# Chlumsky/msdfgen

Measured on AMD Instinct MI355X. Metric: MSDF glyphs/sec (64x64, fp32), higher is better.
Workload: dtype f64

## Files before the change

include/msdfgen_hip.h:

```cpp
#ifndef MSDFGEN_HIP_H
#define MSDFGEN_HIP_H

#include <stddef.h>
#include <stdint.h>

#ifdef __cplusplus
extern "C" {
#endif

#define MSDFHIP_ABI_VERSION 5

#define MSDFHIP_MODE_SDF   1
#define MSDFHIP_MODE_PSDF  2
#define MSDFHIP_MODE_MSDF  3
#define MSDFHIP_MODE_MTSDF 4

#define MSDFHIP_EC_DISABLED       0
#define MSDFHIP_EC_INDISCRIMINATE 1
#define MSDFHIP_EC_EDGE_PRIORITY  2
#define MSDFHIP_EC_EDGE_ONLY      3
#define MSDFHIP_DO_NOT_CHECK_DISTANCE  0
#define MSDFHIP_CHECK_DISTANCE_AT_EDGE 1
#define MSDFHIP_ALWAYS_CHECK_DISTANCE  2

// ... 182 lines not shown
int msdfhip_simulate_8bit_host(float *pixels, int width, int height, int row_stride, int channels);

int msdfhip_set_kernel_timing(int enable);
int msdfhip_kernel_timing(double *avg_ms_distance, double *avg_ms_correction, int *launches, int reset);

int msdfhip_trim(void);

int msdfhip_front_door_devices(int *out, int cap);

int msdfhip_reload_tuning(void);
int msdfhip_debug_wait_profile(unsigned long long *out24, int reset);
int msdfhip_debug_bbcount(unsigned *out, int cap, int reset);
int msdfhip_debug_single_call_phases(double *out8, int reset);

int msdfhip_single_call_fallbacks(unsigned long long *barrier_timeouts, unsigned long long *lost_flags, unsigned long long *refused, int reset);

#define MSDFHIP_ROUTE_DIST_SMALL_SIMPLE      0
#define MSDFHIP_ROUTE_DIST_SMALL_OVERLAP     1
#define MSDFHIP_ROUTE_DIST_ONE_QUAD          2
#define MSDFHIP_ROUTE_DIST_ONE_SINGLE        3
#define MSDFHIP_ROUTE_DIST_LDS_QUAD          4
#define MSDFHIP_ROUTE_DIST_LDS_SINGLE        5
#define MSDFHIP_ROUTE_DIST_GLOBAL_DIRECT     6
#define MSDFHIP_ROUTE_DIST_GLOBAL_PERSISTENT 7
#define MSDFHIP_ROUTE_DIST_FULL_SIMPLE       8
#define MSDFHIP_ROUTE_DIST_UNCULLED          9
#define MSDFHIP_ROUTE_EC_QUERY_HEAVIEST     10
#define MSDFHIP_ROUTE_EC_QUERY_BATCH        11
#define MSDFHIP_ROUTE_EC_WIDE_SLOTS         12
#define MSDFHIP_ROUTE_EC_SLOW_ALL           13
#define MSDFHIP_ROUTE_SIGN_WHOLE_ROWS       14
#define MSDFHIP_ROUTE_SIGN_SPLIT            15
#define MSDFHIP_ROUTE_SIGN_CHUNKED          16
#define MSDFHIP_ROUTE_COUNT                 17
int msdfhip_debug_route_counts(unsigned long long *out, int cap, int reset);

#ifdef __cplusplus
}
#endif
#endif
```

msdfgen_amd/csrc/msdf_capi.hip:

```cpp

#include <hip/hip_runtime.h>

#include <algorithm>
#include <atomic>
#include <chrono>
#include <condition_variable>
#include <cmath>
#include <cstdarg>
#include <cstdio>
#include <cstdlib>
#include <cstring>
#include <deque>
#include <functional>
#include <memory>
#include <mutex>
#include <string>
#include <thread>
#include <vector>

#include <sched.h>

#include "msdf_classplan.hpp"
#include "msdf_hostplan.hpp"
#include "msdf_kernels.hpp"
// ... 11 lines not shown
int fail(int code, const char *fmt, ...) {
    char buf[512];
    va_list ap;
    va_start(ap, fmt);
    vsnprintf(buf, sizeof(buf), fmt, ap);
    va_end(ap);
    tlsError = buf;
    return code;
}


static long long nowNsEarly() { return std::chrono::duration_cast<std::chrono::nanoseconds>(std::chrono::steady_clock::now().time_since_epoch()).count(); }

struct Tuning {
    size_t resLdsBudget;
    long persistentRounds;
    bool serialClasses;
    int querySlotCap, queryLpcContours;
    bool hasQueryLds;
    bool hasQueryPolicy;
    int qpEdgeCost, qpMaxEdges, qpMinCount, qpWideMaxEdges;
    float qpWideLoad, qpWideMeanCount;
    size_t signCap;
    bool pipelineTrace;
    int microbatch;
    int queryStatic;
    int queryGridSteps;
    int queryBatch;
    bool noArgPayloadSingle;
    bool noZeroCopySingle;
    bool noFusedSingle;
    double shareGridFactor;
    long persistentGrid;
    long shortRounds;
    long smallLaunchTiles;
    char devices[256];
    int smallMaxEdges;
    int ldsClassTpw;
    int pipelineDepth;
    bool prepLargeTier;
    int hostThreads;
    long singleSpinLimit;
    bool singleVerbose;
};
std::atomic<const Tuning *> gTuning(NULL);
std::mutex gTuningMutex;
std::vector<Tuning *> gTuningTables;

void readTuning() {
    Tuning &t = *new Tuning;
    const char *env;
    t.resLdsBudget = (env = getenv("MSDFHIP_RES_LDS_BUDGET")) ? (size_t) atol(env) : (size_t) 10*1024;
    t.persistentRounds = (env = getenv("MSDFHIP_PERSISTENT_ROUNDS")) ? atol(env) : 8;
    t.serialClasses = getenv("MSDFHIP_SERIAL_CLASSES") != NULL;
    t.querySlotCap = 160, t.queryLpcContours = 24;
    t.hasQueryLds = (env = getenv("MSDFHIP_QUERY_LDS")) != NULL;
    if (env)
        sscanf(env, "%d,%d", &t.querySlotCap, &t.queryLpcContours);
    t.qpEdgeCost = 150, t.qpMaxEdges = 48, t.qpMinCount = 0x7fffffff, t.qpWideMaxEdges = 128, t.qpWideLoad = 4e8f, t.qpWideMeanCount = 24.f;
    t.hasQueryPolicy = (env = getenv("MSDFHIP_QUERY_POLICY")) != NULL;
    if (env)
        sscanf(env, "%d,%d,%d,%d,%f,%f", &t.qpEdgeCost, &t.qpMaxEdges, &t.qpMinCount, &t.qpWideMaxEdges, &t.qpWideLoad, &t.qpWideMeanCount);
    t.signCap = (env = getenv("MSDFHIP_SIGN_CAP")) ? (size_t) atol(env) : (size_t) 192;
    if (t.signCap < 3)
        t.signCap = 3;
    t.pipelineTrace = getenv("MSDFHIP_PIPELINE_TRACE") != NULL;
    t.microbatch = (env = getenv("MSDFHIP_MICROBATCH")) ? atoi(env) : 256;
    if (t.microbatch < 1)
        t.microbatch = 1;
    t.devices[0] = 0;
    t.queryStatic = (env = getenv("MSDFHIP_QUERY_STATIC")) ? atoi(env) : 2;
    t.queryGridSteps = (env = getenv("MSDFHIP_QUERY_GRID")) ? atoi(env) : 16;
    t.queryBatch = (env = getenv("MSDFHIP_QUERY_BATCH")) && atoi(env) > 0 ? atoi(env) : 1;
    t.noFusedSingle = getenv("MSDFHIP_NO_FUSED_SINGLE") != NULL;
    t.noZeroCopySingle = getenv("MSDFHIP_NO_ZERO_COPY_SINGLE") != NULL;
    t.noArgPayloadSingle = getenv("MSDFHIP_NO_ARG_PAYLOAD_SINGLE") != NULL;
    t.shortRounds = (env = getenv("MSDFHIP_SHORT_ROUNDS")) ? atol(env) : 4;
    t.persistentGrid = (env = getenv("MSDFHIP_PERSISTENT_GRID")) ? atol(env) : 0;
    t.shareGridFactor = (env = getenv("MSDFHIP_SHARE_GRID")) ? atof(env) : 1.33;
    t.smallLaunchTiles = (env = getenv("MSDFHIP_SMALL_LAUNCH_TILES")) ? atol(env) : 8192;
    if ((env = getenv("MSDFHIP_DEVICES")))
        snprintf(t.devices, sizeof(t.devices), "%s", env);
    t.smallMaxEdges = (env = getenv("MSDFHIP_SMALL_MAX_EDGES")) && atoi(env) > 0 ? atoi(env) : 128;
    t.ldsClassTpw = (env = getenv("MSDFHIP_LDS_CLASS_TPW")) && atoi(env) == 1 ? 1 : 4;
    t.pipelineDepth = (env = getenv("MSDFHIP_PIPELINE_DEPTH")) && atoi(env) >= 1 && atoi(env) <= 3 ? atoi(env) : 2;
    t.prepLargeTier = getenv("MSDFHIP_PREP_LARGE_TIER") != NULL;
    t.hostThreads = (env = getenv("MSDFHIP_HOST_THREADS")) && atoi(env) > 0 ? atoi(env) : 0;
    t.singleSpinLimit = (env = getenv("MSDFHIP_SINGLE_SPIN_LIMIT")) && atol(env) > 0 ? atol(env) : 0;
    t.singleVerbose = getenv("MSDFHIP_SINGLE_VERBOSE") != NULL;
    gTuningTables.push_back(&t);
    gTuning.store(&t, std::memory_order_release);
}

const Tuning &tuning() {
    const Tuning *t = gTuning.load(std::memory_order_acquire);
    if (!t) {
        std::lock_guard<std::mutex> lock(gTuningMutex);
        if (!gTuning.load(std::memory_order_acquire))
            readTuning();
        t = gTuning.load(std::memory_order_acquire);
    }
    return *t;
}

std::atomic<unsigned long long> gRouteCounts[MSDFHIP_ROUTE_COUNT];

inline void countRoute(int route) { gRouteCounts[route].fetch_add(1, std::memory_order_relaxed); }

#define HIPCHK(expr) do { hipError_t e_ = (expr); if (e_ != hipSuccess) { (void) hipGetLastError(); return fail(MSDFHIP_ERR_HIP, "%s failed: %s (%s:%d)", #expr, hipGetErrorString(e_), __FILE__, __LINE__); } } while (0)

// ... 99 lines not shown
    WorkBuffer() { }
    WorkBuffer(const WorkBuffer &) = delete;
    WorkBuffer &operator=(const WorkBuffer &) = delete;
    ~WorkBuffer() { release(); }
    void release() {
        if (owned && ptr)
            (void) (PINNED ? pinnedFree(ptr) : hipFree(ptr));
        ptr = NULL, cap = 0, owned = false;
    }
    void borrow(T *p, size_t n) { release(); ptr = p, cap = n; }
    hipError_t ensure(size_t n) {
        if (cap >= n)
            return hipSuccess;
        release();
        const hipError_t e = PINNED ? pinnedAlloc((void **) &ptr, n*sizeof(T)) : hipMalloc((void **) &ptr, n*sizeof(T));
        if (e != hipSuccess) {
            ptr = NULL;
            return e;
        }
        cap = n, owned = true;
        return hipSuccess;
    }
};

struct Workspace {
    int device = 0;
    std::mutex mutex;
    WorkBuffer<float> scratch;
    WorkBuffer<EcCandidate> deferred;
    WorkBuffer<EcGlyphParams> ecParams;
    WorkBuffer<double> gres;
    WorkBuffer<unsigned> workQueue;
    unsigned queueParity = 0;
    WorkBuffer<int> bucket;
    WorkBuffer<int, true> hBucket;
    int bucketKey = -1;
    bool bucketUploaded = false;
    WorkBuffer<int> ecOrder;
    WorkBuffer<int, true> hEcOrder;
    hipEvent_t ecOrderReady = NULL;
    bool ecOrderTried = false;
    hipStream_t sideStream[2] = { NULL, NULL };
    hipEvent_t forkEvent = NULL, joinEvent[2] = { NULL, NULL };

    size_t reservedGlyphs = 0;

    void newGlyphRange() { bucketKey = -1, bucketUploaded = false; }
    void reserveGlyphs(size_t n) {
        bucket.release(), hBucket.release(), ecParams.release();
        reservedGlyphs = n;
        newGlyphRange();
    }
    size_t glyphCapacity(int nGlyphs) const { return std::max(std::max((size_t) (nGlyphs > 0 ? nGlyphs : 0), reservedGlyphs), (size_t) 1); }
    ~Workspace() {
        if (!(scratch.owned || deferred.owned || ecParams.owned || gres.owned || workQueue.owned || bucket.owned || hBucket.owned || ecOrder.owned || hEcOrder.owned ||
              ecOrderReady || forkEvent || sideStream[0] || sideStream[1]))
            return;
        (void) hipSetDevice(device);
        for (int k = 0; k < 2; ++k) {
            if (sideStream[k])
                hipStreamDestroy(sideStream[k]);
            if (joinEvent[k])
                hipEventDestroy(joinEvent[k]);
        }
        if (forkEvent)
            hipEventDestroy(forkEvent);
        if (ecOrderReady)
            hipEventDestroy(ecOrderReady);
    }
};

struct ShapeData {
    int nGlyphs = 0, nContours = 0, nEdges = 0, maxContours = 0, maxEdges = 0;
    int32_t *dGlyphContourOffsets = NULL, *dContourOffsets = NULL;
    double *dPoints = NULL;
    uint8_t *dTypes = NULL, *dColors = NULL;
    EdgeRec *dRecs = NULL;
    int8_t *dWindings = NULL;
    mutable std::vector<int> hContours, hEdges;
    void countMaxima() {
        maxContours = maxEdges = 0;
        for (size_t g = 0; g < hContours.size(); ++g)
            maxContours = std::max(maxContours, hContours[g]), maxEdges = std::max(maxEdges, hEdges[g]);
    }
    void setCounts(const int *contours, const int *edges, int n) {
        hContours.assign(contours, contours+n), hEdges.assign(edges, edges+n);
        countMaxima();
    }
// ... 92 lines not shown
    plan.resBytes = resBytes;
    plan.globalRes = overlap && resBytes+idxBytes > plan.ldsBudget;
    plan.idxBytes = idxBytes;
    plan.listStride = maxEdges;
    plan.bytes = plan.globalRes ? tileListBytes(maxEdges, maxContours, true) : resBytes+idxBytes;
    if (plan.bytes > limit)
        return fail(MSDFHIP_ERR_TOO_COMPLEX, "a glyph has %d contours / %d edges: the survivor lists need %zu B of LDS per wavefront, device limit is %zu B",
                    maxContours, maxEdges, plan.bytes, limit);
    return MSDFHIP_OK;
}

template <class K>
int setLds(K kernel, size_t bytes) {
    if (bytes > 64*1024)
        HIPCHK(hipFuncSetAttribute(reinterpret_cast<const void *>(kernel), hipFuncAttributeMaxDynamicSharedMemorySize, (int) bytes));
    return MSDFHIP_OK;
}

int ensureWorkQueue(const MsdfHipBatch *b, unsigned **out, hipStream_t stream) {
    std::lock_guard<std::mutex> lock(b->work.mutex);
    WorkBuffer<unsigned> &q = b->work.workQueue;
    if (!q.ptr) {
        HIPCHK(q.ensure(64));
        const hipError_t e = hipMemsetAsync(q.ptr, 0, 256, stream);
        if (e != hipSuccess) {
            q.release();
            return fail(MSDFHIP_ERR_HIP, "work queue of the persistent launch: %s", hipGetErrorString(e));
        }
    }
    *out = q.ptr;
    return MSDFHIP_OK;
}

int ensureGres(const MsdfHipBatch *b, size_t bytes, double **out) {
    std::lock_guard<std::mutex> lock(b->work.mutex);
    HIPCHK(b->work.gres.ensure((bytes+sizeof(double)-1)/sizeof(double)));
    *out = b->work.gres.ptr;
    return MSDFHIP_OK;
}

template <int SEL, bool OVERLAP, bool GRES, int TPW_>
void launchDistanceKernel(unsigned grid, size_t lds, hipStream_t stream, const DistanceArgs &a) {
    hipLaunchKernelGGL((k_distance<SEL, OVERLAP, GRES, TPW_>), dim3(grid), dim3(WAVE), lds, stream, a.batch.nGlyphs, a.batch.glyphContourOffsets, a.batch.contourOffsets,
                       a.batch.recs, a.batch.windings, a.glyphs, a.width, a.height, a.tilesX, a.tilesPerGlyph, a.maxEdges, a.dst, a.toScratch, a.blockBase, a.gres,
                       a.gresStride, a.glyphMap, a.nMapped, a.workQueue, a.workItems);
}

template <int SEL, bool OVERLAP, bool GRES, int TPW_ = (GRES ? 1 : (int) QUAD)>
int launchDistance(const MsdfHipBatch *b, const MsdfHipGlyph *dGlyphs, int w, int h, float *dst, int toScratch, const LdsPlan &plan, hipStream_t stream,
                   const int *dGlyphMap = NULL, int nMapped = 0, size_t shareGrid = 0, bool *persistent = NULL) {
    const int tilesX = (w+TILE-1)/TILE, tilesY = (h+TILE-1)/TILE, tiles = tilesX*tilesY;
    if (persistent)
        *persistent = false;
    const int nG = dGlyphMap ? nMapped : b->nGlyphs;
    if (nG == 0)
        return MSDFHIP_OK;
    const int tpw = TPW_;
    const size_t blocks = (size_t) nG*(size_t) ((tiles+tpw-1)/tpw);
    if (blocks > 0x7fffffffull)
        return fail(MSDFHIP_ERR_INVALID, "launch of %zu tile quads exceeds the grid limit; split the batch", blocks);
    int rc = setLds(k_distance<SEL, OVERLAP, GRES, TPW_>, plan.bytes);
    if (rc != MSDFHIP_OK)
        return rc;
    double *gres = NULL;
    size_t chunk = blocks, stride = 0;
    unsigned *queue = NULL;
    DistanceArgs args;
    args.batch = viewOf(b), args.glyphs = dGlyphs, args.width = w, args.height = h, args.tilesX = tilesX, args.tilesPerGlyph = tiles, args.maxEdges = plan.listStride;
    args.dst = dst, args.toScratch = toScratch, args.blockBase = 0, args.gres = NULL, args.gresStride = 0, args.glyphMap = dGlyphMap, args.nMapped = nMapped;
    args.workQueue = NULL, args.workItems = 0;
    if (GRES && OVERLAP && plan.resBytes) {
        stride = plan.resBytes/sizeof(double);
        const size_t slots = (size_t) residentSlots(b->device)*4u*MSDF_DISTANCE_WAVES_PER_SIMD;
        const size_t minRounds = (size_t) tuning().persistentRounds;
        const bool byShare = shareGrid > 0 && shareGrid < slots && blocks > shareGrid;
        if (((minRounds && blocks >= minRounds*slots) || byShare) && blocks < 0xffffffffull-8u*slots) {
            chunk = byShare ? shareGrid : slots;
            if (tuning().persistentGrid > 0 && (size_t) tuning().persistentGrid < chunk)
                chunk = (size_t) tuning().persistentGrid;
            rc = ensureGres(b, chunk*plan.resBytes, &gres);
            if (rc == MSDFHIP_OK)
                rc = ensureWorkQueue(b, &queue, stream);
            if (rc != MSDFHIP_OK)
                return rc;
            std::lock_guard<std::mutex> lock(b->work.mutex);
            queue += b->work.queueParity ? 16 : 0;
            args.gres = gres, args.gresStride = stride, args.workQueue = queue, args.workItems = (unsigned) blocks;
            launchDistanceKernel<SEL, OVERLAP, GRES, TPW_>((unsigned) chunk, plan.bytes, stream, args);
            HIPCHK(hipGetLastError());
            b->work.queueParity ^= 1u;
            if (persistent)
                *persistent = true;
            return MSDFHIP_OK;
        }
        chunk = GRES_WORKSPACE_CAP/plan.resBytes;
        if (chunk < 256)
            chunk = 256;
        if (chunk > blocks)
            chunk = blocks;
        rc = ensureGres(b, chunk*plan.resBytes, &gres);
        if (rc != MSDFHIP_OK)
            return rc;
    }
// ... 245 lines not shown
            return rc;
        HIPCHK(hipEventRecord(b->work.forkEvent, stream));
        if (nRest > 0 && b->plan.nSmall > 0) {
            sRest = b->work.sideStream[0];
            HIPCHK(hipStreamWaitEvent(sRest, b->work.forkEvent, 0));
        }
        if (b->plan.nOne > 0 && (b->plan.nSmall > 0 || nRest > 0)) {
            sOne = b->work.sideStream[1];
            HIPCHK(hipStreamWaitEvent(sOne, b->work.forkEvent, 0));
        }
    }
    int aheadRc = MSDFHIP_OK;
    if (ecAhead && sOne != stream) {
        aheadRc = runCorrection(b, SelTraits<SEL>::NCH, w, h, dGlyphs, NULL, NULL, NULL, *ecAhead, sOne, call, true);
    }
    if (nRest > 0) {
        LdsPlan rest = plan;
        rest.globalRes = true;
        rest.bytes = tileListBytes(maxE, maxC, true);
        size_t shareGrid = 0;
        if (tuning().shareGridFactor > 0 && concurrent) {
            const size_t slots = (size_t) residentSlots(b->device)*4u*MSDF_DISTANCE_WAVES_PER_SIMD;
            shareGrid = (size_t) ((double) slots*b->plan.restShare*tuning().shareGridFactor);
            shareGrid = shareGrid < 256 ? 256 : shareGrid;
        }
        rc = launchDistance<SEL, true, true>(b, dGlyphs, w, h, dst, toScratch, rest, sRest, b->work.bucket.ptr+b->plan.nOne+b->plan.nSmall, nRest, shareGrid, &persistent);
        rc = counted(rc, persistent ? MSDFHIP_ROUTE_DIST_GLOBAL_PERSISTENT : MSDFHIP_ROUTE_DIST_GLOBAL_DIRECT);
    }
    if (rc == MSDFHIP_OK && b->plan.nSmall > 0) {
        const size_t slots = (size_t) residentSlots(b->device)*4u*MSDF_DISTANCE_WAVES_PER_SIMD;
        const bool shortLaunch = classTpw == 1 || (size_t) b->plan.nSmall*(size_t) ((tilesAll+QUAD-1)/QUAD) < (size_t) tuning().shortRounds*slots;
        LdsPlan small;
        rc = planLds(b, SelTraits<SEL>::NCH, true, small, b->plan.smallMaxC, b->plan.smallMaxE, shortLaunch ? 1 : (int) QUAD);
        if (rc == MSDFHIP_OK)
            rc = shortLaunch ? counted(launchDistance<SEL, true, false, 1>(b, dGlyphs, w, h, dst, toScratch, small, stream, b->work.bucket.ptr+b->plan.nOne, b->plan.nSmall),
                                       MSDFHIP_ROUTE_DIST_LDS_SINGLE)
                             : counted(launchDistance<SEL, true, false>(b, dGlyphs, w, h, dst, toScratch, small, stream, b->work.bucket.ptr+b->plan.nOne, b->plan.nSmall),
                                       MSDFHIP_ROUTE_DIST_LDS_QUAD);
    }
    if (rc == MSDFHIP_OK && b->plan.nOne > 0) {
        const size_t slots = (size_t) residentSlots(b->device)*4u*MSDF_SIMPLE_WAVES_PER_SIMD;
        const bool shortLaunch = (size_t) b->plan.nOne*(size_t) ((tilesAll+QUAD-1)/QUAD) < (size_t) tuning().shortRounds*slots;
        LdsPlan simple;
        rc = planLds(b, SelTraits<SEL>::NCH, false, simple, 1, b->plan.oneMaxE, shortLaunch ? 1 : (int) QUAD);
        if (rc == MSDFHIP_OK && shortLaunch) {
            simple.bytes = tileListBytes(b->plan.oneMaxE, 1, true);
            rc = counted(launchDistance<SEL, false, true>(b, dGlyphs, w, h, dst, toScratch, simple, sOne, b->work.bucket.ptr, b->plan.nOne), MSDFHIP_ROUTE_DIST_ONE_SINGLE);
        } else if (rc == MSDFHIP_OK)
            rc = counted(launchDistance<SEL, false, false>(b, dGlyphs, w, h, dst, toScratch, simple, sOne, b->work.bucket.ptr, b->plan.nOne), MSDFHIP_ROUTE_DIST_ONE_QUAD);
    }
    hipError_t joinError = hipSuccess;
    if (sRest != stream) {
        hipError_t e = hipEventRecord(b->work.joinEvent[0], sRest);
        if (e == hipSuccess)
            e = hipStreamWaitEvent(stream, b->work.joinEvent[0], 0);
        joinError = e != hipSuccess ? e : joinError;
    }
    if (sOne != stream) {
        hipError_t e = hipEventRecord(b->work.joinEvent[1], sOne);
        if (e == hipSuccess)
            e = hipStreamWaitEvent(stream, b->work.joinEvent[1], 0);
        joinError = e != hipSuccess ? e : joinError;
    }
    rc = aheadRc != MSDFHIP_OK ? aheadRc : rc;
    if (joinError != hipSuccess) {
        (void) hipGetLastError();
        if (sRest != stream)
            (void) hipStreamSynchronize(sRest);
        if (sOne != stream)
            (void) hipStreamSynchronize(sOne);
        if (rc == MSDFHIP_OK)
// ... 3165 lines not shown
```

msdfgen_amd/csrc/msdf_classplan.hpp:

```cpp

#pragma once

#include <algorithm>
#include <cstddef>

namespace msdfhip {

inline size_t tileListBytes(int maxEdges, int maxContours, bool withBounds) { return ((size_t) maxEdges+(withBounds ? 4 : 1)*(size_t) maxContours+2)*sizeof(int); }

const int SMALL_MAX_EDGES = 128;
const int COST_LDS_MAX_CONTOURS = 5;

inline double glyphCost(int contours, int edges) {
    static const double kOne[4] = { 0.25625, 0.01190, 0.00000, 0.00000 }, kLds[4] = { 0.38398, 0.00846, -0.02755, 0.003446 }, kGlobal[4] = { 1.11611, 0.015776, -0.05039, 0.000681 };
    const double *k = contours <= 1 ? kOne : (contours <= COST_LDS_MAX_CONTOURS && edges <= SMALL_MAX_EDGES) ? kLds : kGlobal;
    const double c = k[0]+k[1]*edges+k[2]*contours+k[3]*(double) edges*contours;
    return c > k[0] ? c : k[0];
}

struct ClassPlan {
    int nOne = 0, nSmall = 0, nHuge = 0;
    int oneMaxE = 0, smallMaxC = 0, smallMaxE = 0, restMaxC = 0, restMaxE = 0;
    float restShare = 1.f;
};

inline ClassPlan planClasses(const int *contours, const int *edges, int n, int limit, int smallMaxEdges, size_t ldsLimit, int *order) {
    auto classOf = [=](int g) {
        if (tileListBytes(edges[g], contours[g], true) > ldsLimit)
            return 3;
        return contours[g] <= 1 ? 0 : contours[g] <= limit && edges[g] <= smallMaxEdges ? 1 : 2;
    };
    int end[4], maxC[4] = { 0, 0, 0, 0 }, maxE[4] = { 0, 0, 0, 0 }, at = 0;
    for (int k = 0; k < 4; ++k) {
        for (int g = 0; g < n; ++g)
            if (classOf(g) == k) {
                order[at++] = g;
                maxC[k] = std::max(maxC[k], contours[g]), maxE[k] = std::max(maxE[k], edges[g]);
            }
        end[k] = at;
    }
    auto heavier = [=](int x, int y) { return (long long) edges[x]*std::max(contours[x], 1) > (long long) edges[y]*std::max(contours[y], 1); };
    for (int k = 0; k < 3; ++k)
        std::stable_sort(order+(k ? end[k-1] : 0), order+end[k], heavier);
    double all = 0, rest = 0;
    for (int g = 0; g < n; ++g)
        all += glyphCost(contours[g], edges[g]);
    for (int k = end[1]; k < end[2]; ++k)
        rest += glyphCost(contours[order[k]], edges[order[k]]);
    ClassPlan p;
    p.nOne = end[0], p.nSmall = end[1]-end[0], p.nHuge = end[3]-end[2];
    p.oneMaxE = maxE[0], p.smallMaxC = maxC[1], p.smallMaxE = maxE[1], p.restMaxC = maxC[2], p.restMaxE = maxE[2];
    p.restShare = all > 0 ? (float) (rest/all) : 1.f;
    return p;
}

}
```

msdfgen_amd/csrc/msdf_kernels.hpp:

```cpp
#pragma once

#include <hip/hip_runtime.h>
#include "msdf_device.hpp"
#include "msdf_prep.hpp"
#include "msdf_ec.hpp"
#include "msdf_ec_fast.hpp"
#include "msdf_cull.hpp"
#include "msdf_scanline.hpp"
#include "msdf_shapeprep.hpp"
#include "msdf_frame.hpp"
#include "../../include/msdfgen_hip.h"

namespace msdfhip {

#ifndef MSDF_DISTANCE_WAVES_PER_SIMD
#define MSDF_DISTANCE_WAVES_PER_SIMD 4
#endif
constexpr int TILE = 8;
constexpr int WAVE = 64;
constexpr int REC_DOUBLES = sizeof(EdgeRec)/sizeof(double);

struct BatchView {
    int nGlyphs;
    const int32_t *glyphContourOffsets;
// ... 112 lines not shown
__device__ inline GlyphWork decodeItem(unsigned b, int nGlyphs, int tilesPerGlyph) {
    GlyphWork w;
    const unsigned fullBlocks = ((unsigned) nGlyphs&~7u)*(unsigned) tilesPerGlyph;
    if (b >= fullBlocks) {
        const unsigned j = b-fullBlocks;
        w.g = (int) (((unsigned) nGlyphs&~7u)+j/(unsigned) tilesPerGlyph);
        w.tile = (int) (j%(unsigned) tilesPerGlyph);
    } else {
        const unsigned xcd = b&7u, slot = b>>3;
        w.g = (int) ((slot/(unsigned) tilesPerGlyph)*8u+xcd);
        w.tile = (int) (slot%(unsigned) tilesPerGlyph);
    }
    w.valid = w.g < nGlyphs;
    return w;
}
__device__ inline GlyphWork decodeBlock(int nGlyphs, int tilesPerGlyph, unsigned blockBase = 0) {
    return decodeItem(blockIdx.x+blockBase, nGlyphs, tilesPerGlyph);
}

__device__ inline unsigned nextItem(unsigned *counters, unsigned total, int &steal) {
    const unsigned x = blockIdx.x&7u;
    while (steal < 8) {
        const unsigned xx = (x+(unsigned) steal)&7u;
        unsigned k = 0;
        if (threadIdx.x == 0)
            k = atomicAdd(&counters[xx], 1u);
        k = (unsigned) __builtin_amdgcn_readfirstlane((int) k);
        const unsigned b = k*8u+xx;
        if (b < total)
            return b;
        ++steal;
    }
    return ~0u;
}

__device__ inline Xform loadXform(const MsdfHipGlyph &gd) {
    Xform t;
    t.sx = gd.xf[0], t.sy = gd.xf[1], t.tx = gd.xf[2], t.ty = gd.xf[3];
    t.mapScale = gd.xf[4], t.mapTranslate = gd.xf[5];
    return t;
}

__device__ inline void stageRecords(double *dst, const EdgeRec *src, int n) {
    const double *s = reinterpret_cast<const double *>(src);
    const int total = n*REC_DOUBLES;
    for (int i = threadIdx.x; i < total; i += blockDim.x)
        dst[i] = s[i];
}


__device__ inline void waveSync() {
    __builtin_amdgcn_fence(__ATOMIC_RELEASE, "wavefront");
    __builtin_amdgcn_wave_barrier();
    __builtin_amdgcn_fence(__ATOMIC_ACQUIRE, "wavefront");
}

__device__ inline float waveMinNonNegative(float v) {
    int x = __float_as_int(v);
    const int inf = 0x7f800000;
#define MSDF_DPP_MIN(ctrl, rowmask) { const int y = __builtin_amdgcn_update_dpp(inf, x, ctrl, rowmask, 0xf, false); x = y < x ? y : x; }
    MSDF_DPP_MIN(0x111, 0xf)
    MSDF_DPP_MIN(0x112, 0xf)
    MSDF_DPP_MIN(0x114, 0xf)
    MSDF_DPP_MIN(0x118, 0xf)
    MSDF_DPP_MIN(0x142, 0xa)
    MSDF_DPP_MIN(0x143, 0xc)
// ... 273 lines not shown
        __syncthreads();
        if (rank == 0)
            for (int r = 1; r < TEAM; ++r) {
                Selector<SEL> other;
                teamGet(other, x+(size_t) (r-1)*TEAM_XCHG_DOUBLES*WAVE, lane);
                selMergePartial(s, other);
            }
        __syncthreads();
        return rank == 0;
    }
    __device__ bool isHelper() const { return rank != 0; }
};

enum { QUAD = 4 };

#ifndef MSDF_SIMPLE_WAVES_PER_SIMD
#define MSDF_SIMPLE_WAVES_PER_SIMD 5
#endif
struct DistanceArgs {
    BatchView batch;
    const MsdfHipGlyph *glyphs;
    int width, height, tilesX, tilesPerGlyph, maxEdges;
    float *dst;
    int toScratch;
    unsigned blockBase;
    double *gres;
    size_t gresStride;
    const int *glyphMap;
    int nMapped;
    unsigned *workQueue;
    unsigned workItems;
};

template <int SEL, bool OVERLAP, bool GRES, int TPW_ = (GRES ? 1 : (int) QUAD), int TEAM = 1>
__device__ __forceinline__ void distanceBody(int nGlyphs, const int32_t *__restrict__ glyphContourOffsets, const int32_t *__restrict__ contourOffsets, const EdgeRec *__restrict__ recs,
           const int8_t *__restrict__ windings, const MsdfHipGlyph *__restrict__ glyphs, int width, int height, int tilesX, int tilesPerGlyph, int maxEdges,
           float *__restrict__ dst, int toScratch, unsigned blockBase, double *__restrict__ gres, size_t gresStride, const int *__restrict__ glyphMap, int nMapped,
           unsigned *__restrict__ workQueue, unsigned workItems, const unsigned blockId, double *smem, const int knownContours = -1, const int knownEdges = -1,
           double *teamXchg = NULL) {
    static_assert(TEAM == 1 || (TPW_ == 1 && !GRES), "teams take one tile, combiner scratch in LDS");
    const int teamRank = TEAM > 1 ? MSDF_UNIFORM((int) (threadIdx.x>>6)) : 0;
    enum { NCH = SelTraits<SEL>::NCH, TPW = TPW_, ROW = WAVE/TPW };
    BatchView batch;
    batch.nGlyphs = nGlyphs, batch.glyphContourOffsets = glyphContourOffsets, batch.contourOffsets = contourOffsets, batch.recs = recs, batch.windings = windings;
    unsigned item = blockId+blockBase;
    int steal = 0;
    const bool persistent = GRES && workQueue != NULL;
    for (;;) {
    if (persistent) {
        item = nextItem(workQueue, workItems, steal);
        if (item == ~0u) {
            if (blockId == 0 && threadIdx.x < 8)
                reinterpret_cast<unsigned *>(reinterpret_cast<size_t>(workQueue)^64u)[threadIdx.x] = 0u;
            return;
        }
    }
    const int quadsPerGlyph = (tilesPerGlyph+TPW-1)/TPW;
    GlyphWork wk = decodeItem(item, glyphMap ? nMapped : batch.nGlyphs, quadsPerGlyph);
    if (!wk.valid)
        return;
    if (glyphMap)
        wk.g = MSDF_UNIFORM(glyphMap[wk.g]);
    const int c0 = knownContours >= 0 ? 0 : MSDF_UNIFORM(batch.glyphContourOffsets[wk.g]), C = knownContours >= 0 ? knownContours : MSDF_UNIFORM(batch.glyphContourOffsets[wk.g+1])-c0;
    const int32_t *coff = batch.contourOffsets+c0;
    const int e0 = knownContours >= 0 ? 0 : MSDF_UNIFORM(coff[0]);
    const int lane = TEAM > 1 ? (int) (threadIdx.x&(WAVE-1)) : (int) threadIdx.x;
    const EdgeRec *rec = batch.recs+e0;

    double *res = GRES ? gres+(size_t) blockId*gresStride : smem;
    int *lists = reinterpret_cast<int *>(smem+(OVERLAP && !GRES ? (size_t) C*NCH*WAVE : 0));
    int *cstarts = lists+(size_t) TPW*maxEdges;

    const MsdfHipGlyph gd = glyphs[wk.g];
    const Xform t = loadXform(gd);
    WindingMasks wind;
    wind.mem = batch.windings+c0;
    if (OVERLAP) {
        const int w = lane < C ? (int) wind.mem[lane] : 0;
        wind.pos = __ballot(w > 0), wind.neg = __ballot(w < 0);
    }
#if defined(MSDF_PROFILE_WAITS)
    MSDF_STAMP(pStart);
    unsigned long long pAcc[16] = { 0, 0, 0, 0, 0, 0, 0, 0, 0, 0, 0, 0, 0, 0, 0, 0 };
#endif

    const double rsx = 1/t.sx, rsy = 1/t.sy;
    const bool fastXf = divSafe(t.sx) && divSafe(t.sy);
    const double hx = (.5*TILE-.5)*fabs(rsx), hy = (.5*TILE-.5)*fabs(rsy);
    const double tr = sqrt(hx*hx+hy*hy);
    if (TEAM == 1 || teamRank == 0) {
        const int q = lane/ROW, col = lane%ROW;
// ... 161 lines not shown
#if defined(__HIP_DEVICE_COMPILE__)
        asm volatile("" : "+v"(laneAfter));
#endif
        const int xo = tx*TILE+(laneAfter&(TILE-1)), yo = ty*TILE+(laneAfter>>3);
        const int yn = gd.flip ? height-1-yo : yo;
        float *px = toScratch ? dst+(((size_t) wk.g*height+yn)*width+xo)*NCH
                              : dst+gd.out_offset+(ptrdiff_t) gd.row_stride*yn+(ptrdiff_t) NCH*xo;
        for (int ch = 0; ch < NCH; ++ch) {
            __builtin_nontemporal_store(mapDistance(t, d[ch]), &px[ch]);
        }
#if defined(MSDF_PROFILE_WAITS)
        {
            MSDF_STAMP(tTile1);
            edges.prof[13] += tTile1-tTile0;
        }
        for (int i = 0; i < 16; ++i)
            pAcc[i] += edges.prof[i];
#endif
    }
#if defined(MSDF_PROFILE_WAITS)
    {
        MSDF_STAMP(pEnd);
        if (lane == 0) {
            atomicAdd(&gWaitProfile[0], 1ull), atomicAdd(&gWaitProfile[1], pEnd-pStart), atomicAdd(&gWaitProfile[2], pPhase2-pStart);
            atomicAdd(&gWaitProfile[3], pAcc[0]), atomicAdd(&gWaitProfile[4], pAcc[1]), atomicAdd(&gWaitProfile[5], pAcc[2]), atomicAdd(&gWaitProfile[6], pAcc[3]);
            atomicAdd(&gWaitProfile[7], pAcc[4]), atomicAdd(&gWaitProfile[8], pAcc[5]), atomicAdd(&gWaitProfile[9], pAcc[6]), atomicAdd(&gWaitProfile[10], pEnd-pPhase2);
            atomicAdd(&gWaitProfile[11], pAcc[7]&0xffffffffull), atomicAdd(&gWaitProfile[12], pAcc[7]>>32);
            atomicAdd(&gWaitProfile[13], pAcc[8]), atomicAdd(&gWaitProfile[14], pAcc[9]), atomicAdd(&gWaitProfile[15], pAcc[10]);
            atomicAdd(&gWaitProfile[16], pAcc[11]), atomicAdd(&gWaitProfile[17], pAcc[13]);
            atomicAdd(&gWaitProfile[18], pAcc[14]), atomicAdd(&gWaitProfile[19], pAcc[15]);
        }
    }
#endif
    if (!persistent)
        return;
    waveSync();
    }
}

template <int SEL, bool OVERLAP, bool GRES = false, int TPW_ = (GRES ? 1 : (int) QUAD)>
__global__ void __launch_bounds__(WAVE, OVERLAP ? MSDF_DISTANCE_WAVES_PER_SIMD : GRES ? MSDF_SIMPLE_WAVES_PER_SIMD-1 : MSDF_SIMPLE_WAVES_PER_SIMD)
k_distance(int nGlyphs, const int32_t *__restrict__ glyphContourOffsets, const int32_t *__restrict__ contourOffsets, const EdgeRec *__restrict__ recs,
           const int8_t *__restrict__ windings, const MsdfHipGlyph *__restrict__ glyphs, int width, int height, int tilesX, int tilesPerGlyph, int maxEdges,
           float *__restrict__ dst, int toScratch, unsigned blockBase, double *__restrict__ gres, size_t gresStride, const int *__restrict__ glyphMap, int nMapped,
           unsigned *__restrict__ workQueue, unsigned workItems) {
    extern __shared__ __attribute__((aligned(16))) double smem[];
    distanceBody<SEL, OVERLAP, GRES, TPW_>(nGlyphs, glyphContourOffsets, contourOffsets, recs, windings, glyphs, width, height, tilesX, tilesPerGlyph, maxEdges, dst, toScratch, blockBase,
                                     gres, gresStride, glyphMap, nMapped, workQueue, workItems, blockIdx.x, smem);
}


template <bool OVERLAP, class Wind = const int8_t *, class Edges = EdgesAll>
struct PsdfQuery {
    const EdgeRec *rec;
    const int32_t *coff;
    Wind windings;
    int C;
    double *res;
    __device__ double operator()(V2 q) const {
        double out[1];
        Edges edges;
        edges.coff = coff;
        if (OVERLAP)
            shapeDistanceOverlap<2>(rec, edges, windings, C, q, res, WAVE, out);
        else
            shapeDistanceSimple<2>(rec, edges, C, q, out);
        return out[0];
    }
};

typedef PB PBSlot;

struct EdgesCooperative {
    const int32_t *coff;
    int lane;
    PBSlot *slots;
    PBSlot *merged;
    int nE, C;
    mutable unsigned long long cached;
    int cacheCap;
// ... 1271 lines not shown
```

msdfgen_amd/lib.py:

```python
import ctypes as C
import os
import threading

import numpy as np

from . import build as _build

MODE_SDF, MODE_PSDF, MODE_MSDF, MODE_MTSDF = 1, 2, 3, 4
CHANNELS = {1: 1, 2: 1, 3: 3, 4: 4}
EC_DISABLED, EC_INDISCRIMINATE, EC_EDGE_PRIORITY, EC_EDGE_ONLY = 0, 1, 2, 3
DO_NOT_CHECK_DISTANCE, CHECK_DISTANCE_AT_EDGE, ALWAYS_CHECK_DISTANCE = 0, 1, 2
FILL_NONZERO, FILL_ODD, FILL_POSITIVE, FILL_NEGATIVE = 0, 1, 2, 3
ERR_NO_DEVICE, ERR_INVALID, ERR_HIP, ERR_TOO_COMPLEX, ERR_NOMEM = -1, -2, -3, -4, -5

_dp = C.POINTER(C.c_double)
_ip = C.POINTER(C.c_int32)
_fp = C.POINTER(C.c_float)
_bp = C.POINTER(C.c_uint8)
_vp = C.c_void_p


class MsdfHipError(RuntimeError):
    def __init__(self, code, message):
        super().__init__("msdfgen_hip error %d: %s" % (code, message))
# ... 84 lines not shown
    "msdfhip_front_door_devices": (C.c_int, [C.POINTER(C.c_int), C.c_int]),
    "msdfhip_debug_wait_profile": (C.c_int, [C.POINTER(C.c_ulonglong), C.c_int]),
    "msdfhip_debug_single_call_phases": (C.c_int, [C.POINTER(C.c_double), C.c_int]),
    "msdfhip_debug_bbcount": (C.c_int, [C.POINTER(C.c_uint32), C.c_int, C.c_int]),
    "msdfhip_generate_stream": (C.c_int, [C.c_int, C.c_int, C.c_int, C.c_int, C.c_int, _vp, _vp, _vp, C.c_size_t, _vp, C.c_size_t, _vp, C.POINTER(Config)]),
    "msdfhip_generate_stream_csr": (C.c_int, [C.c_int, C.c_int, C.c_int, C.c_int, C.c_int, _ip, _ip, _dp, _bp, _bp, _vp, _vp, C.c_size_t, _vp, C.c_size_t, _vp,
                                              C.POINTER(Config)]),
    "msdfhip_generate_stream_prepared": (C.c_int, [C.c_int, C.c_int, C.c_int, C.c_int, C.c_int, _vp, _vp, _vp, C.c_size_t, _vp, C.c_size_t, _vp, C.POINTER(Config),
                                                   C.POINTER(PrepConfig), C.POINTER(C.c_uint64)]),
    "msdfhip_generate_stream_csr_prepared": (C.c_int, [C.c_int, C.c_int, C.c_int, C.c_int, C.c_int, _ip, _ip, _dp, _bp, _bp, _vp, _vp, C.c_size_t, _vp, C.c_size_t,
                                                       _vp, C.POINTER(Config), C.POINTER(PrepConfig), C.POINTER(C.c_uint64)]),
    "msdfhip_generate_stream_prepared_oriented": (C.c_int, [C.c_int, C.c_int, C.c_int, C.c_int, C.c_int, _vp, _vp, _vp, C.c_size_t, _vp, C.c_size_t, _vp,
                                                            C.POINTER(Config), C.POINTER(PrepConfig), C.POINTER(C.c_uint64), C.POINTER(OrientConfig)]),
    "msdfhip_generate_stream_csr_prepared_oriented": (C.c_int, [C.c_int, C.c_int, C.c_int, C.c_int, C.c_int, _ip, _ip, _dp, _bp, _bp, _vp, _vp, C.c_size_t, _vp,
                                                                C.c_size_t, _vp, C.POINTER(Config), C.POINTER(PrepConfig), C.POINTER(C.c_uint64),
                                                                C.POINTER(OrientConfig)]),
    "msdfhip_batch_bounds": (C.c_int, [_vp, _dp]),
    "msdfhip_batch_frame": (C.c_int, [_vp, C.POINTER(FrameConfig), C.c_int, C.c_int, _vp, _vp]),
    "msdfhip_generate_stream_prepared_oriented_framed": (C.c_int, [C.c_int, C.c_int, C.c_int, C.c_int, C.c_int, _vp, _vp, _vp, C.c_size_t, _vp, C.c_size_t, _vp,
                                                                   C.POINTER(Config), C.POINTER(PrepConfig), C.POINTER(C.c_uint64), C.POINTER(OrientConfig),
                                                                   C.POINTER(FrameConfig)]),
    "msdfhip_generate_stream_csr_prepared_oriented_framed": (C.c_int, [C.c_int, C.c_int, C.c_int, C.c_int, C.c_int, _ip, _ip, _dp, _bp, _bp, _vp, _vp, C.c_size_t,
                                                                       _vp, C.c_size_t, _vp, C.POINTER(Config), C.POINTER(PrepConfig), C.POINTER(C.c_uint64),
                                                                       C.POINTER(OrientConfig), C.POINTER(FrameConfig)]),
    "msdfhip_set_host_threads": (C.c_int, [C.c_int]),
    "msdfhip_single_call_fallbacks": (C.c_int, [C.POINTER(C.c_ulonglong), C.POINTER(C.c_ulonglong), C.POINTER(C.c_ulonglong), C.c_int]),
    "msdfhip_debug_route_counts": (C.c_int, [C.POINTER(C.c_ulonglong), C.c_int, C.c_int]),
}

EXPORTED_SYMBOLS = tuple(sorted(_PROTOS))

ROUTE_NAMES = ("dist_small_simple", "dist_small_overlap", "dist_one_quad", "dist_one_single", "dist_lds_quad", "dist_lds_single", "dist_global_direct",
               "dist_global_persistent", "dist_full_simple", "dist_unculled", "ec_query_heaviest", "ec_query_batch", "ec_wide_slots", "ec_slow_all",
               "sign_whole_rows", "sign_split", "sign_chunked")

_lib = None
_lock = threading.Lock()


def library_path():
    return _build.LIB


def load(build_if_missing=True):
    global _lib
    with _lock:
        if _lib is not None:
            return _lib
        try:
            import torch
        except ImportError:
            pass
        path = os.environ.get("MSDFGEN_HIP_LIB") or _build.LIB
        if path == _build.LIB and not os.path.exists(path):
            if not build_if_missing:
                raise MsdfHipError(ERR_NO_DEVICE, "libmsdfgen_hip.so is not built (python -m msdfgen_amd.build)")
            _build.build_lib()
        lib = C.CDLL(path)
        for name, (restype, argtypes) in _PROTOS.items():
            fn = getattr(lib, name)
            fn.restype = restype
            fn.argtypes = argtypes
        if lib.msdfhip_abi_version() != 5:
            raise MsdfHipError(ERR_INVALID, "ABI version mismatch")
        _lib = lib
        return lib

# ... 50 lines not shown
```

Measured before the change: 1.732 million.

## Add glyph-affine persistent scheduling for the LDS quad distance kernel

Adds a persistent launch mode for the LDS-class quad distance kernel. Each wave reads its XCC and CU hardware ids and pulls tiles from per-XCC, per-home-CU atomic counters, so tiles of the same glyph land on the same CU or XCC and reuse its cached edge data. A one-time probe kernel maps the live CU slots to homes, and waves that run out of local work steal from other XCCs using a ballot over counters. In exchange it adds atomic contention, a probe launch on first use, and reliance on hardware register layouts; small launches keep the old path through a round-count threshold.

```diff
diff --git a/include/msdfgen_hip.h b/include/msdfgen_hip.h
--- a/include/msdfgen_hip.h
+++ b/include/msdfgen_hip.h
@@ -238,7 +238,8 @@
 #define MSDFHIP_ROUTE_SIGN_WHOLE_ROWS       14
 #define MSDFHIP_ROUTE_SIGN_SPLIT            15
 #define MSDFHIP_ROUTE_SIGN_CHUNKED          16
-#define MSDFHIP_ROUTE_COUNT                 17
+#define MSDFHIP_ROUTE_DIST_LDS_AFFINE        17
+#define MSDFHIP_ROUTE_COUNT                 18
 int msdfhip_debug_route_counts(unsigned long long *out, int cap, int reset);
 
 #ifdef __cplusplus
diff --git a/msdfgen_amd/csrc/msdf_capi.hip b/msdfgen_amd/csrc/msdf_capi.hip
--- a/msdfgen_amd/csrc/msdf_capi.hip
+++ b/msdfgen_amd/csrc/msdf_capi.hip
@@ -67,6 +67,10 @@
     bool noFusedSingle;
     double shareGridFactor;
     long persistentGrid;
+    int affineMode;
+    long affineRounds;
+    double affineGridFactor;
+    int affineHomeCus;
     long shortRounds;
     long smallLaunchTiles;
     char devices[256];
@@ -111,6 +115,10 @@
     t.noZeroCopySingle = getenv("MSDFHIP_NO_ZERO_COPY_SINGLE") != NULL;
     t.noArgPayloadSingle = getenv("MSDFHIP_NO_ARG_PAYLOAD_SINGLE") != NULL;
     t.shortRounds = (env = getenv("MSDFHIP_SHORT_ROUNDS")) ? atol(env) : 4;
+    t.affineMode = (env = getenv("MSDFHIP_AFFINE")) ? (atoi(env) != 0 ? 1 : 0) : -1;
+    t.affineRounds = (env = getenv("MSDFHIP_AFFINE_ROUNDS")) && atol(env) >= 0 ? atol(env) : 8;
+    t.affineGridFactor = (env = getenv("MSDFHIP_AFFINE_GRID")) && atof(env) > 0 ? atof(env) : 1.0;
+    t.affineHomeCus = (env = getenv("MSDFHIP_AFFINE_HOME")) && !strcmp(env, "pair") ? 2 : 1;
     t.persistentGrid = (env = getenv("MSDFHIP_PERSISTENT_GRID")) ? atol(env) : 0;
     t.shareGridFactor = (env = getenv("MSDFHIP_SHARE_GRID")) ? atof(env) : 1.33;
     t.smallLaunchTiles = (env = getenv("MSDFHIP_SMALL_LAUNCH_TILES")) ? atol(env) : 8192;
@@ -276,6 +284,9 @@
     WorkBuffer<double> gres;
     WorkBuffer<unsigned> workQueue;
     unsigned queueParity = 0;
+    WorkBuffer<unsigned> affineQueue;
+    unsigned affineParity = 0;
+    int affineHomeCus = 0;
     WorkBuffer<int> bucket;
     WorkBuffer<int, true> hBucket;
     int bucketKey = -1;
@@ -297,7 +308,7 @@
     }
     size_t glyphCapacity(int nGlyphs) const { return std::max(std::max((size_t) (nGlyphs > 0 ? nGlyphs : 0), reservedGlyphs), (size_t) 1); }
     ~Workspace() {
-        if (!(scratch.owned || deferred.owned || ecParams.owned || gres.owned || workQueue.owned || bucket.owned || hBucket.owned || ecOrder.owned || hEcOrder.owned ||
+        if (!(scratch.owned || deferred.owned || ecParams.owned || gres.owned || workQueue.owned || affineQueue.owned || bucket.owned || hBucket.owned || ecOrder.owned || hEcOrder.owned ||
               ecOrderReady || forkEvent || sideStream[0] || sideStream[1]))
             return;
         (void) hipSetDevice(device);
@@ -456,6 +467,82 @@
     return MSDFHIP_OK;
 }
 
+struct Placement {
+    int homes[2] = { 0, 0 };
+    uint8_t table[2][AFFINE_PLACEMENT_SLOTS];
+};
+const Placement *placementOf(int device) {
+    static std::mutex mutex;
+    static Placement *known[64];
+    if (device < 0 || device >= 64)
+        return NULL;
+    std::lock_guard<std::mutex> lock(mutex);
+    if (known[device])
+        return known[device];
+    Placement *p = new Placement;
+    known[device] = p;
+    memset(p->table, 0, sizeof(p->table));
+    uint8_t *dSeen = NULL;
+    hipStream_t s = NULL;
+    std::vector<uint8_t> seen((size_t) AFFINE_PLACEMENT_SLOTS, 0);
+    bool ok = hipMalloc((void **) &dSeen, AFFINE_PLACEMENT_SLOTS) == hipSuccess && hipStreamCreateWithFlags(&s, hipStreamNonBlocking) == hipSuccess &&
+              hipMemsetAsync(dSeen, 0, AFFINE_PLACEMENT_SLOTS, s) == hipSuccess;
+    if (ok) {
+        hipLaunchKernelGGL(k_probe_placement, dim3((unsigned) residentSlots(device)*64u), dim3(WAVE), 0, s, dSeen);
+        ok = hipGetLastError() == hipSuccess && hipMemcpyAsync(seen.data(), dSeen, AFFINE_PLACEMENT_SLOTS, hipMemcpyDeviceToHost, s) == hipSuccess &&
+             hipStreamSynchronize(s) == hipSuccess;
+    }
+    if (s)
+        (void) hipStreamDestroy(s);
+    if (dSeen)
+        (void) hipFree(dSeen);
+    if (!ok) {
+        (void) hipGetLastError();
+        return p;
+    }
+    int fewest = AFFINE_MAX_HOMES;
+    for (int x = 0; x < 8; ++x) {
+        int n = 0;
+        for (int k = 0; k < 256; ++k)
+            n += seen[(size_t) x*256+k] != 0;
+        fewest = std::min(fewest, n);
+    }
+    if (fewest < 1)
+        return p;
+    for (int pair = 0; pair < 2; ++pair) {
+        const int H = pair ? (fewest+1)/2 : fewest;
+        for (int x = 0; x < 8; ++x)
+            for (int k = 0, rank = 0; k < 256; ++k) {
+                const bool live = seen[(size_t) x*256+k] != 0;
+                p->table[pair][(size_t) x*256+k] = (uint8_t) ((live ? (pair ? rank/2 : rank) : k)%H);
+                rank += live;
+            }
+        p->homes[pair] = H;
+    }
+    return p;
+}
+
+int ensureAffineQueue(const MsdfHipBatch *b, const Placement *p, int homeCus, unsigned **out, hipStream_t stream) {
+    std::lock_guard<std::mutex> lock(b->work.mutex);
+    WorkBuffer<unsigned> &q = b->work.affineQueue;
+    if (!q.ptr) {
+        HIPCHK(q.ensure(AFFINE_QUEUE_WORDS));
+        b->work.affineHomeCus = 0, b->work.affineParity = 0;
+        const hipError_t e = hipMemsetAsync(q.ptr, 0, sizeof(unsigned)*2*AFFINE_SET_WORDS, stream);
+        if (e != hipSuccess) {
+            q.release();
+            return fail(MSDFHIP_ERR_HIP, "work queues of the glyph-affine launch: %s", hipGetErrorString(e));
+        }
+    }
+    if (b->work.affineHomeCus != homeCus) {
+        HIPCHK(hipMemcpyAsync(q.ptr+2*AFFINE_SET_WORDS, p->table[homeCus == 2], AFFINE_PLACEMENT_SLOTS, hipMemcpyHostToDevice, stream));
+        HIPCHK(hipMemsetAsync(q.ptr, 0, sizeof(unsigned)*2*AFFINE_SET_WORDS, stream));
+        b->work.affineHomeCus = homeCus;
+    }
+    *out = q.ptr;
+    return MSDFHIP_OK;
+}
+
 int ensureGres(const MsdfHipBatch *b, size_t bytes, double **out) {
     std::lock_guard<std::mutex> lock(b->work.mutex);
     HIPCHK(b->work.gres.ensure((bytes+sizeof(double)-1)/sizeof(double)));
@@ -463,9 +550,9 @@
     return MSDFHIP_OK;
 }
 
-template <int SEL, bool OVERLAP, bool GRES, int TPW_>
+template <int SEL, bool OVERLAP, bool GRES, int TPW_, bool AFFINE = false>
 void launchDistanceKernel(unsigned grid, size_t lds, hipStream_t stream, const DistanceArgs &a) {
-    hipLaunchKernelGGL((k_distance<SEL, OVERLAP, GRES, TPW_>), dim3(grid), dim3(WAVE), lds, stream, a.batch.nGlyphs, a.batch.glyphContourOffsets, a.batch.contourOffsets,
+    hipLaunchKernelGGL((k_distance<SEL, OVERLAP, GRES, TPW_, AFFINE>), dim3(grid), dim3(WAVE), lds, stream, a.batch.nGlyphs, a.batch.glyphContourOffsets, a.batch.contourOffsets,
                        a.batch.recs, a.batch.windings, a.glyphs, a.width, a.height, a.tilesX, a.tilesPerGlyph, a.maxEdges, a.dst, a.toScratch, a.blockBase, a.gres,
                        a.gresStride, a.glyphMap, a.nMapped, a.workQueue, a.workItems);
 }
@@ -493,6 +580,26 @@
     args.batch = viewOf(b), args.glyphs = dGlyphs, args.width = w, args.height = h, args.tilesX = tilesX, args.tilesPerGlyph = tiles, args.maxEdges = plan.listStride;
     args.dst = dst, args.toScratch = toScratch, args.blockBase = 0, args.gres = NULL, args.gresStride = 0, args.glyphMap = dGlyphMap, args.nMapped = nMapped;
     args.workQueue = NULL, args.workItems = 0;
+    if (!GRES && OVERLAP && TPW_ == (int) QUAD && shareGrid > 0) {
+        const int homeCus = tuning().affineHomeCus;
+        const Placement *p = placementOf(b->device);
+        const int H = p ? p->homes[homeCus == 2] : 0;
+        if (H > 0 && H <= (int) AFFINE_MAX_HOMES) {
+            rc = ensureAffineQueue(b, p, homeCus, &queue, stream);
+            if (rc == MSDFHIP_OK)
+                rc = setLds(k_distance<SEL, OVERLAP, GRES, TPW_, (!GRES && OVERLAP && TPW_ == (int) QUAD)>, plan.bytes);
+            if (rc != MSDFHIP_OK)
+                return rc;
+            std::lock_guard<std::mutex> lock(b->work.mutex);
+            args.workQueue = queue, args.workItems = (unsigned) H|(b->work.affineParity<<8);
+            launchDistanceKernel<SEL, OVERLAP, GRES, TPW_, (!GRES && OVERLAP && TPW_ == (int) QUAD)>((unsigned) std::min(shareGrid, blocks), plan.bytes, stream, args);
+            HIPCHK(hipGetLastError());
+            b->work.affineParity ^= 1u;
+            if (persistent)
+                *persistent = true;
+            return MSDFHIP_OK;
+        }
+    }
     if (GRES && OVERLAP && plan.resBytes) {
         stride = plan.resBytes/sizeof(double);
         const size_t slots = (size_t) residentSlots(b->device)*4u*MSDF_DISTANCE_WAVES_PER_SIMD;
@@ -804,11 +911,23 @@
         const bool shortLaunch = classTpw == 1 || (size_t) b->plan.nSmall*(size_t) ((tilesAll+QUAD-1)/QUAD) < (size_t) tuning().shortRounds*slots;
         LdsPlan small;
         rc = planLds(b, SelTraits<SEL>::NCH, true, small, b->plan.smallMaxC, b->plan.smallMaxE, shortLaunch ? 1 : (int) QUAD);
-        if (rc == MSDFHIP_OK)
-            rc = shortLaunch ? counted(launchDistance<SEL, true, false, 1>(b, dGlyphs, w, h, dst, toScratch, small, stream, b->work.bucket.ptr+b->plan.nOne, b->plan.nSmall),
-                                       MSDFHIP_ROUTE_DIST_LDS_SINGLE)
-                             : counted(launchDistance<SEL, true, false>(b, dGlyphs, w, h, dst, toScratch, small, stream, b->work.bucket.ptr+b->plan.nOne, b->plan.nSmall),
-                                       MSDFHIP_ROUTE_DIST_LDS_QUAD);
+        if (rc == MSDFHIP_OK && shortLaunch)
+            rc = counted(launchDistance<SEL, true, false, 1>(b, dGlyphs, w, h, dst, toScratch, small, stream, b->work.bucket.ptr+b->plan.nOne, b->plan.nSmall),
+                         MSDFHIP_ROUTE_DIST_LDS_SINGLE);
+        else if (rc == MSDFHIP_OK) {
+            size_t affineGrid = 0;
+            if (tuning().affineMode != 0) {
+                affineGrid = (size_t) ((double) slots*(concurrent ? b->plan.smallShare : 1.f)*tuning().affineGridFactor);
+                affineGrid = std::min(std::max(affineGrid, (size_t) 256), slots);
+                if (tuning().affineMode < 0 && (size_t) b->plan.nSmall*(size_t) ((tilesAll+QUAD-1)/QUAD) < (size_t) tuning().affineRounds*affineGrid)
+                    affineGrid = 0;
+            }
+            bool affine = false;
+            rc = launchDistance<SEL, true, false>(b, dGlyphs, w, h, dst, toScratch, small, stream, b->work.bucket.ptr+b->plan.nOne, b->plan.nSmall, affineGrid, &affine);
+            rc = counted(rc, MSDFHIP_ROUTE_DIST_LDS_QUAD);
+            if (affine)
+                rc = counted(rc, MSDFHIP_ROUTE_DIST_LDS_AFFINE);
+        }
     }
     if (rc == MSDFHIP_OK && b->plan.nOne > 0) {
         const size_t slots = (size_t) residentSlots(b->device)*4u*MSDF_SIMPLE_WAVES_PER_SIMD;
diff --git a/msdfgen_amd/csrc/msdf_classplan.hpp b/msdfgen_amd/csrc/msdf_classplan.hpp
--- a/msdfgen_amd/csrc/msdf_classplan.hpp
+++ b/msdfgen_amd/csrc/msdf_classplan.hpp
@@ -22,6 +22,7 @@
     int nOne = 0, nSmall = 0, nHuge = 0;
     int oneMaxE = 0, smallMaxC = 0, smallMaxE = 0, restMaxC = 0, restMaxE = 0;
     float restShare = 1.f;
+    float smallShare = 1.f;
 };
 
 inline ClassPlan planClasses(const int *contours, const int *edges, int n, int limit, int smallMaxEdges, size_t ldsLimit, int *order) {
@@ -42,15 +43,18 @@
     auto heavier = [=](int x, int y) { return (long long) edges[x]*std::max(contours[x], 1) > (long long) edges[y]*std::max(contours[y], 1); };
     for (int k = 0; k < 3; ++k)
         std::stable_sort(order+(k ? end[k-1] : 0), order+end[k], heavier);
-    double all = 0, rest = 0;
+    double all = 0, rest = 0, small = 0;
     for (int g = 0; g < n; ++g)
         all += glyphCost(contours[g], edges[g]);
     for (int k = end[1]; k < end[2]; ++k)
         rest += glyphCost(contours[order[k]], edges[order[k]]);
+    for (int k = end[0]; k < end[1]; ++k)
+        small += glyphCost(contours[order[k]], edges[order[k]]);
     ClassPlan p;
     p.nOne = end[0], p.nSmall = end[1]-end[0], p.nHuge = end[3]-end[2];
     p.oneMaxE = maxE[0], p.smallMaxC = maxC[1], p.smallMaxE = maxE[1], p.restMaxC = maxC[2], p.restMaxE = maxE[2];
     p.restShare = all > 0 ? (float) (rest/all) : 1.f;
+    p.smallShare = all > 0 ? (float) (small/all) : 1.f;
     return p;
 }
 
diff --git a/msdfgen_amd/csrc/msdf_kernels.hpp b/msdfgen_amd/csrc/msdf_kernels.hpp
--- a/msdfgen_amd/csrc/msdf_kernels.hpp
+++ b/msdfgen_amd/csrc/msdf_kernels.hpp
@@ -168,6 +168,60 @@
         ++steal;
     }
     return ~0u;
+}
+
+enum { AFFINE_MAX_HOMES = 64, AFFINE_COUNTER_WORDS = 16, AFFINE_SET_WORDS = 8*AFFINE_MAX_HOMES*AFFINE_COUNTER_WORDS, AFFINE_PLACEMENT_SLOTS = 8*256,
+       AFFINE_QUEUE_WORDS = 2*AFFINE_SET_WORDS+AFFINE_PLACEMENT_SLOTS/4 };
+
+__device__ inline unsigned placementSlot() {
+    const unsigned xcc = __builtin_amdgcn_s_getreg(20|(3<<11))&7u;
+    const unsigned cu = __builtin_amdgcn_s_getreg(4|(8<<6)|(7<<11));
+    return xcc<<8|cu;
+}
+
+__device__ inline bool nextAffineItem(unsigned *set, const uint8_t *table, unsigned H, unsigned nGlyphs, unsigned quads, unsigned &state, GlyphWork &wk) {
+    if (state == ~0u) {
+        const unsigned slot = placementSlot();
+        state = (slot>>8)*H+table[slot];
+    }
+    for (;;) {
+        const unsigned cur = state&0xffffu, x = cur/H, l = cur-x*H;
+        const unsigned nx = (nGlyphs+7u-x)>>3;
+        const unsigned limit = (nx/H+(l < nx%H ? 1u : 0u))*quads;
+        unsigned k = 0;
+        if (threadIdx.x == 0)
+            k = atomicAdd(&set[cur*AFFINE_COUNTER_WORDS], 1u);
+        k = (unsigned) __builtin_amdgcn_readfirstlane((int) k);
+        if (k < limit) {
+            const unsigned m = k/quads;
+            wk.g = (int) (x+8u*(l+m*H)), wk.tile = (int) (k-m*quads), wk.valid = true;
+            return true;
+        }
+        const unsigned own = placementSlot(), l0 = table[own];
+        unsigned steal = state>>16;
+        bool found = false;
+        for (; steal < 8u; ++steal) {
+            const unsigned xx = ((own>>8)+steal)&7u, nxx = (nGlyphs+7u-xx)>>3, q = nxx/H, r = nxx-q*H;
+            bool live = false;
+            if (threadIdx.x < H)
+                live = __hip_atomic_load(&set[(xx*H+threadIdx.x)*AFFINE_COUNTER_WORDS], __ATOMIC_RELAXED, __HIP_MEMORY_SCOPE_AGENT) < (q+(threadIdx.x < r ? 1u : 0u))*quads;
+            const unsigned long long any = __ballot(live), after = any&(~0ull<<l0);
+            if (any) {
+                state = steal<<16|(xx*H+(unsigned) (__ffsll((unsigned long long) (after ? after : any))-1));
+                found = true;
+                break;
+            }
+        }
+        if (!found)
+            return false;
+    }
+}
+
+__global__ void k_probe_placement(uint8_t *__restrict__ seen) {
+    const unsigned slot = placementSlot();
+    __builtin_amdgcn_s_sleep(127);
+    if (threadIdx.x == 0 && slot < (unsigned) AFFINE_PLACEMENT_SLOTS)
+        seen[slot] = 1;
 }
 
 __device__ inline Xform loadXform(const MsdfHipGlyph &gd) {
@@ -507,7 +561,7 @@
     unsigned workItems;
 };
 
-template <int SEL, bool OVERLAP, bool GRES, int TPW_ = (GRES ? 1 : (int) QUAD), int TEAM = 1>
+template <int SEL, bool OVERLAP, bool GRES, int TPW_ = (GRES ? 1 : (int) QUAD), int TEAM = 1, bool AFFINE = false>
 __device__ __forceinline__ void distanceBody(int nGlyphs, const int32_t *__restrict__ glyphContourOffsets, const int32_t *__restrict__ contourOffsets, const EdgeRec *__restrict__ recs,
            const int8_t *__restrict__ windings, const MsdfHipGlyph *__restrict__ glyphs, int width, int height, int tilesX, int tilesPerGlyph, int maxEdges,
            float *__restrict__ dst, int toScratch, unsigned blockBase, double *__restrict__ gres, size_t gresStride, const int *__restrict__ glyphMap, int nMapped,
@@ -521,6 +575,12 @@
     unsigned item = blockId+blockBase;
     int steal = 0;
     const bool persistent = GRES && workQueue != NULL;
+    static_assert(!AFFINE || (OVERLAP && !GRES && TEAM == 1 && TPW_ == (int) QUAD), "the glyph-affine queue serves the LDS class's quad form");
+    const bool affine = AFFINE;
+    unsigned affineState = ~0u;
+    if (affine && blockId == 0)
+        for (unsigned i = threadIdx.x; i < 8u*(workItems&0xffu); i += WAVE)
+            workQueue[(size_t) (~workItems>>8&1u)*AFFINE_SET_WORDS+(size_t) i*AFFINE_COUNTER_WORDS] = 0u;
     for (;;) {
     if (persistent) {
         item = nextItem(workQueue, workItems, steal);
@@ -531,7 +591,13 @@
         }
     }
     const int quadsPerGlyph = (tilesPerGlyph+TPW-1)/TPW;
-    GlyphWork wk = decodeItem(item, glyphMap ? nMapped : batch.nGlyphs, quadsPerGlyph);
+    GlyphWork wk;
+    if (affine) {
+        if (!nextAffineItem(workQueue+(size_t) (workItems>>8&1u)*AFFINE_SET_WORDS, reinterpret_cast<const uint8_t *>(workQueue+2*AFFINE_SET_WORDS), workItems&0xffu,
+                            (unsigned) (glyphMap ? nMapped : batch.nGlyphs), (unsigned) quadsPerGlyph, affineState, wk))
+            return;
+    } else
+        wk = decodeItem(item, glyphMap ? nMapped : batch.nGlyphs, quadsPerGlyph);
     if (!wk.valid)
         return;
     if (glyphMap)
@@ -759,20 +825,20 @@
         }
     }
 #endif
-    if (!persistent)
+    if (!persistent && !affine)
         return;
     waveSync();
     }
 }
 
-template <int SEL, bool OVERLAP, bool GRES = false, int TPW_ = (GRES ? 1 : (int) QUAD)>
+template <int SEL, bool OVERLAP, bool GRES = false, int TPW_ = (GRES ? 1 : (int) QUAD), bool AFFINE = false>
 __global__ void __launch_bounds__(WAVE, OVERLAP ? MSDF_DISTANCE_WAVES_PER_SIMD : GRES ? MSDF_SIMPLE_WAVES_PER_SIMD-1 : MSDF_SIMPLE_WAVES_PER_SIMD)
 k_distance(int nGlyphs, const int32_t *__restrict__ glyphContourOffsets, const int32_t *__restrict__ contourOffsets, const EdgeRec *__restrict__ recs,
            const int8_t *__restrict__ windings, const MsdfHipGlyph *__restrict__ glyphs, int width, int height, int tilesX, int tilesPerGlyph, int maxEdges,
            float *__restrict__ dst, int toScratch, unsigned blockBase, double *__restrict__ gres, size_t gresStride, const int *__restrict__ glyphMap, int nMapped,
            unsigned *__restrict__ workQueue, unsigned workItems) {
     extern __shared__ __attribute__((aligned(16))) double smem[];
-    distanceBody<SEL, OVERLAP, GRES, TPW_>(nGlyphs, glyphContourOffsets, contourOffsets, recs, windings, glyphs, width, height, tilesX, tilesPerGlyph, maxEdges, dst, toScratch, blockBase,
+    distanceBody<SEL, OVERLAP, GRES, TPW_, 1, AFFINE>(nGlyphs, glyphContourOffsets, contourOffsets, recs, windings, glyphs, width, height, tilesX, tilesPerGlyph, maxEdges, dst, toScratch, blockBase,
                                      gres, gresStride, glyphMap, nMapped, workQueue, workItems, blockIdx.x, smem);
 }
 
diff --git a/msdfgen_amd/lib.py b/msdfgen_amd/lib.py
--- a/msdfgen_amd/lib.py
+++ b/msdfgen_amd/lib.py
@@ -140,7 +140,7 @@
 
 ROUTE_NAMES = ("dist_small_simple", "dist_small_overlap", "dist_one_quad", "dist_one_single", "dist_lds_quad", "dist_lds_single", "dist_global_direct",
                "dist_global_persistent", "dist_full_simple", "dist_unculled", "ec_query_heaviest", "ec_query_batch", "ec_wide_slots", "ec_slow_all",
-               "sign_whole_rows", "sign_split", "sign_chunked")
+               "sign_whole_rows", "sign_split", "sign_chunked", "dist_lds_affine")
 
 _lib = None
 _lock = threading.Lock()
```

Result: slower. 1.636 million (-5.5%).
